# grant-froelich/Bathymetric-GNN

Measured on AMD Instinct MI355X. Metric: classified tile-nodes/s (fused graph build + 4-layer GAT forward + scatter), higher is better.
Workload: dtype f32

## Files before the change

bathymetric-gnn_amd/csrc/bgnn_api.hip:

```cpp
#include <stdarg.h>
#include <string.h>
#include <stdlib.h>

#include <algorithm>
#include <cmath>

#include "bgnn_internal.h"

namespace bgnn {

static thread_local char g_err[1024] = "";

void set_error(const char *fmt, ...) {
  va_list ap;
  va_start(ap, fmt);
  vsnprintf(g_err, sizeof(g_err), fmt, ap);
  va_end(ap);
}

int DevPool::alloc(size_t bytes, void **out) {
  if (bytes == 0) bytes = 256;
  bytes = (bytes + 255) & ~(size_t)255;
  auto it = free_blocks.lower_bound(bytes);
  if (it != free_blocks.end() && it->first <= bytes + bytes / 4 + 4096) {
// ... 211 lines not shown
    }
    c->owns_stream = true;
  }
  if (hipMalloc((void **)&c->zero_page, 16384) != hipSuccess || hipMemset(c->zero_page, 0, 16384) != hipSuccess) {
    set_error("zero page allocation failed");
    delete c;
    return BGNN_ERR_NOMEM;
  }
  c->stamps = reinterpret_cast<unsigned long long *>(c->zero_page + 1024);
  {
    auto env_int = [](const char *name, int dflt) { const char *e = getenv(name); return e ? atoi(e) : dflt; };
    BgnnOpts &o = c->opts;
    o.matrix_path = getenv("BGNN_BF16") ? 3 : getenv("BGNN_SPLIT_F16") ? 2 : getenv("BGNN_SPLIT_BF16") ? 1 : 0;
    o.fused = getenv("BGNN_NO_FUSED") ? 0 : 1;
    o.fold_extractor = getenv("BGNN_NO_FOLD") ? 0 : 1;
    o.ragged_atlas = getenv("BGNN_NO_ATLAS") ? 0 : 1;
    o.fused_front = getenv("BGNN_NO_FUSED_FRONT") ? 0 : 1;
    o.bf16_two_phase = getenv("BGNN_NO_TWO_PHASE") ? 0 : env_int("BGNN_TWO_PHASE", 1);
    o.bf16_layer0_af = getenv("BGNN_NO_LAYER0_AF") ? 0 : 1;
    o.stats_narrow = env_int("BGNN_STATS_NARROW", -1);
    o.diag_mask = env_int("BGNN_FUSED_DBG", 0);
    o.diag_stamps = getenv("BGNN_FUSED_STAMPS") ? 1 : 0;
    o.gemm_diag = env_int("BGNN_GEMM_DBG", 0);
    o.gemm_pair_major = getenv("BGNN_NO_PAIR_MAJOR") ? 0 : 1;
  }
  *out = c;
  return BGNN_OK;
}

static int *option_slot(bgnn_ctx *ctx, const char *name) {
  BgnnOpts &o = ctx->opts;
  struct { const char *n; int *p; } tab[] = {
      {"matrix_path", &o.matrix_path}, {"fused", &o.fused}, {"fold_extractor", &o.fold_extractor}, {"ragged_atlas", &o.ragged_atlas}, {"features_tiled", &o.features_tiled}, {"fused_front", &o.fused_front}, {"bf16_two_phase", &o.bf16_two_phase}, {"bf16_layer0_af", &o.bf16_layer0_af}, {"stats_narrow", &o.stats_narrow},
      {"diag_mask", &o.diag_mask}, {"diag_stamps", &o.diag_stamps}, {"gemm_diag", &o.gemm_diag}, {"gemm_pair_major", &o.gemm_pair_major}};
  for (auto &t : tab) if (strcmp(t.n, name) == 0) return t.p;
  return nullptr;
}

int bgnn_ctx_set_option(bgnn_ctx *ctx, const char *name, int value) {
  BGNN_REQUIRE(ctx && name, "bgnn_ctx_set_option: NULL argument");
  int *p = option_slot(ctx, name);
  BGNN_REQUIRE(p, "bgnn_ctx_set_option: unknown option '%s'", name);
  if (p == &ctx->opts.matrix_path) BGNN_REQUIRE(value >= 0 && value <= 3, "matrix_path=%d (0 exact f32, 1 bf16x3, 2 fp16x3, 3 bf16 storage)", value);
  if ((p == &ctx->opts.diag_mask || p == &ctx->opts.diag_stamps || p == &ctx->opts.gemm_diag) && value != 0)
    BGNN_REQUIRE(BGNN_DIAG, "option '%s' needs the diagnostic build of the library (python __graft_entry__.py --diag)", name);
  *p = value;
  return BGNN_OK;
}

int bgnn_ctx_get_option(bgnn_ctx *ctx, const char *name, int *value) {
  BGNN_REQUIRE(ctx && name && value, "bgnn_ctx_get_option: NULL argument");
  int *p = option_slot(ctx, name);
  BGNN_REQUIRE(p, "bgnn_ctx_get_option: unknown option '%s'", name);
  *value = *p;
  return BGNN_OK;
}

int bgnn_debug_stamps(bgnn_ctx *ctx, unsigned long long *out32) {
  if (!ctx || !out32) return BGNN_ERR_INVALID;
  (void)hipStreamSynchronize(ctx->stream);
  if (hipMemcpy(out32, ctx->stamps, 512, hipMemcpyDeviceToHost) != hipSuccess) return BGNN_ERR_HIP;
  (void)hipMemset(ctx->stamps, 0, 512);
  return BGNN_OK;
}

int bgnn_ctx_destroy(bgnn_ctx *ctx) {
  if (!ctx) return BGNN_OK;
// ... 285 lines not shown
```

bathymetric-gnn_amd/csrc/bgnn_internal.h:

```cpp
#pragma once
#include <hip/hip_runtime.h>
#include <stdint.h>
#include <stdio.h>
#include <string>
#include <cstdlib>
#include <vector>
#include <map>
#include <set>
#include <atomic>

#include "../../include/bgnn.h"
#include "../../include/bgnn_train.h"
#include "../../include/bgnn_optim.h"
#include "model_images.h"
#include "graph_plan.h"

namespace bgnn {

void set_error(const char *fmt, ...);

#define BGNN_HIP_CHECK(expr)                                                          \
  do {                                                                                \
    hipError_t _e = (expr);                                                           \
    if (_e != hipSuccess) {                                                           \
// ... 17 lines not shown
    if (_r != BGNN_OK) return _r; \
  } while (0)

struct DevPool {
  std::multimap<size_t, void *> free_blocks;
  std::map<void *, size_t> live;
  size_t total_bytes = 0;
  int alloc(size_t bytes, void **out);
  void release(void *p);
  void trim();
};

struct ProfRecord {
  int kernel;
  hipEvent_t start, stop;
};

}

struct BgnnOpts {
  int matrix_path = 0;
  int fused = 1;
  int fold_extractor = 1;
  int bf16_two_phase = 1;
  int bf16_layer0_af = 1;
  int stats_narrow = -1;
  int fused_front = 1;
  int features_tiled = 1;
  int ragged_atlas = 1;
  int diag_mask = 0;
  int diag_stamps = 0;
  int gemm_diag = 0;
  int gemm_pair_major = 1;
};

#ifndef BGNN_DIAG
#define BGNN_DIAG 0
#endif

struct bgnn_ctx {
  int device = 0;
  BgnnOpts opts;
  hipStream_t stream = nullptr;
  bool owns_stream = false;
  bgnn::DevPool pool;
  uint32_t prof_mask = 0;
  std::vector<bgnn::ProfRecord> prof_records;
  std::vector<hipEvent_t> event_pool;
  void *ws[7] = {nullptr, nullptr, nullptr, nullptr, nullptr, nullptr, nullptr};
  size_t ws_bytes[7] = {0, 0, 0, 0, 0, 0, 0};
  struct Staging { void *p; size_t cap; hipEvent_t ev; bool in_flight; };
  std::vector<Staging> staging;
  struct TableCache { int32_t n_tiles, h, w, item_cells; double rx, ry; BgnnTileMeta *d_tiles; BgnnWorkItem *d_items; int32_t n_items; uint64_t stamp; uint64_t id; int32_t refs; };
  std::vector<TableCache> table_cache;
  uint64_t table_stamp = 0, table_next_id = 1;
  std::set<struct bgnn_graph *> live_graphs;
  int num_cus = 256;
  float *zero_page = nullptr;
  unsigned long long *stamps = nullptr;
};

struct BgnnLayer {
  int d_in, heads, width;
  int concat;
  float *Wt;
  float *Wt_blk = nullptr;
// ... 272 lines not shown
```

bathymetric-gnn_amd/csrc/gat_layer_fused.hip:

```cpp
#include <stdlib.h>
#include <algorithm>
#include <type_traits>
#include <utility>
#include "gat_tile_common.h"

namespace bgnn {

typedef float f32x16 __attribute__((ext_vector_type(16)));

enum { EPI_NEXT = 0, EPI_HEADS = 1 };

#if BGNN_DIAG
#define DBG(bit) (a.dbg & (bit))
#define BGNN_STAMP(slot)                                                                   \
  if (a.stamps) {                                                                          \
    const unsigned long long _t = __builtin_amdgcn_s_memtime();                            \
    t_sum[slot] += _t - t_prev;                                                            \
    t_prev = _t;                                                                           \
  }
#else
#define DBG(bit) false
#define BGNN_STAMP(slot)
#endif

// ... 298 lines not shown
template <int KB0, int NB, bool ZERO, bool TAILZ>
__device__ __forceinline__ void agg_blocks(f32x16 &d, uint32_t tr0, uint32_t tr1, uint32_t bq, int hl) {
  u32x2 a0[NB], a1[NB];
  u32x4 b[NB];
#pragma unroll
  for (int i = 0; i < NB; ++i) {
    if (KB0 + i == 0) { a0[i] = lds_read_tr<0>(tr0); a1[i] = lds_read_tr<0>(tr1); b[i] = lds_read4u<0>(bq); }
    if (KB0 + i == 1) { a0[i] = lds_read_tr<1024>(tr0); a1[i] = lds_read_tr<1024>(tr1); b[i] = lds_read4u<32>(bq); }
    if (KB0 + i == 2) { a0[i] = lds_read_tr<2048>(tr0); a1[i] = lds_read_tr<2048>(tr1); b[i] = lds_read4u<64>(bq); }
    if (KB0 + i == 3) { a0[i] = lds_read_tr<3072>(tr0); a1[i] = lds_read_tr<3072>(tr1); b[i] = lds_read4u<96>(bq); }
    if (KB0 + i == 4) { a0[i] = lds_read_tr<4096>(tr0); a1[i] = lds_read_tr<4096>(tr1); b[i] = lds_read4u<128>(bq); }
    if (KB0 + i == 5) { a0[i] = lds_read_tr<5120>(tr0); a1[i] = lds_read_tr<5120>(tr1); b[i] = lds_read4u<160>(bq); }
    if (KB0 + i == 6) { a0[i] = lds_read_tr<6144>(tr0); a1[i] = lds_read_tr<6144>(tr1); b[i] = lds_read4u<192>(bq); }
    if (KB0 + i == 7) { a0[i] = lds_read_tr<7168>(tr0); a1[i] = lds_read_tr<7168>(tr1); b[i] = lds_read4u<224>(bq); }
  }
  lds_reads_done();
#pragma unroll
  for (int i = 0; i < NB; ++i) {
    if (TAILZ && KB0 + i == 7) {
      const u32x4 z4 = {0u, 0u, 0u, 0u};
      if (hl) b[i] = z4;
    }
    const u32x4 av = {a0[i].x, a0[i].y, a1[i].x, a1[i].y};
    const bf16x8 A = __builtin_bit_cast(bf16x8, av), B = __builtin_bit_cast(bf16x8, b[i]);
    if (ZERO && i == 0) {
      const f32x16 z = {0.f, 0.f, 0.f, 0.f, 0.f, 0.f, 0.f, 0.f, 0.f, 0.f, 0.f, 0.f, 0.f, 0.f, 0.f, 0.f};
      d = __builtin_amdgcn_mfma_f32_32x32x16_bf16(A, B, z, 0, 0, 0);
    } else {
      d = __builtin_amdgcn_mfma_f32_32x32x16_bf16(A, B, d, 0, 0, 0);
    }
  }
}

template <int HC, int C, int K, int NT, int EPI, int SP>
struct FusedLds {
  static constexpr int H = HC / C, NC = NT * 32, HR = FusedGeom<K>::HR;
  static constexpr int XB = SP == 3 ? 2 : 4;
  static constexpr int SLAB1 = HR * 32 * XB / 4;
  static constexpr int RING = SP == 3 && NT == 8 && EPI == EPI_NEXT ? 1 : 0;
  static constexpr bool DBUF = RING == 1, WDB = RING == 2;
  static constexpr int SLAB = DBUF ? 2 * SLAB1 : SLAB1;
  static constexpr int WBUF = (WDB ? 4 : 2) * WHalf<NT, SP>::BYTES / 4;
  static constexpr int PATCH_PAD = EPI == EPI_NEXT && SLAB + WBUF < 4 * 32 * TILED_PITCH ? 4 * 32 * TILED_PITCH - SLAB - WBUF : 0;
  static constexpr int HEADW = 96 + 6 * 32 + 8;
  static constexpr bool HAS_IN_ALPHA = SP == 3, HEADW_LATE = SP == 3 && EPI == EPI_HEADS, HID_IN_ALPHA = DBUF || WDB, ATT_LATE = DBUF || WDB;
  static constexpr int ATT_OFF = SLAB1 + 128 > 4 * 32 * TILED_PITCH ? SLAB1 + 128 : 4 * 32 * TILED_PITCH;
  static constexpr int RA = HAS_IN_ALPHA ? 0 : HR * (H + 1), RB = 2 * HC + (EPI == EPI_NEXT ? (ATT_LATE ? 0 : 2 * NC) : HEADW_LATE ? 0 : HEADW);
  static constexpr int RSZ = RA > RB ? RA : RB;
  static constexpr int APITCH = (H * (K + 1)) | 1;
  static constexpr int ALPHA = SP == 3 ? 4 * 32 * AggWindow<K>::PITCH / 4 : 128 * APITCH;
  static_assert(!HAS_IN_ALPHA || HR * (H + 1) + (HID_IN_ALPHA ? HR : 0) <= ALPHA, "the alpha_src and depth tables (and the halo ids) fit the dense-alpha region");
  static_assert(!DBUF || (4 * 32 * TILED_PITCH <= ATT_OFF && ATT_OFF + 2 * NC <= SLAB), "patches | att vectors share the slab region");
  static_assert(!WDB || (4 * 32 * TILED_PITCH <= ATT_OFF && ATT_OFF + 2 * NC <= SLAB + WBUF / 2), "patches | att vectors fit slab + W chunk buffer 0");
  static_assert(!HEADW_LATE || HEADW <= SLAB, "the heads' weight table fits the slab region");
  static_assert(SP != 3 || !AggWindow<K>::TAIL_BEYOND_PITCH || WBUF * 4 >= 8 * 64, "the 8 rows read past the slab image stay inside the W buffer");
  static constexpr int PRE = SLAB + WBUF + PATCH_PAD + RSZ + (HID_IN_ALPHA ? 128 : HR) + 4;
  static constexpr int ALIGN = (4 - PRE % 4) % 4;
  static constexpr int FLOATS = PRE + ALIGN + ALPHA;
  static constexpr bool WIDE_PHASE_A = K == 16 && EPI == EPI_HEADS && SP == 0;
  static constexpr int PER_CU = FLOATS * 4 * 3 <= 160 * 1024 && NT <= 3 && !WIDE_PHASE_A ? 3 : FLOATS * 4 * 2 <= 160 * 1024 ? 2 : 1;
};

template <int HC, int C, int K, int NT, int EPI, int SP = 0, int AGG = 0>
__global__ __launch_bounds__(256, (AGG != 0 && K == 16 ? 2 : FusedLds<HC, C, K, NT, EPI, SP>::PER_CU)) void gat_layer_fused_kernel(FusedArgs a) {
  static_assert(AGG == 0 || (SP == 0 && EPI == EPI_NEXT), "the plain backbones run on the exact path, layer form");
  static_assert(AGG != 2 || HC == 2 * C, "GraphSAGE: two virtual heads");
  constexpr int SRCW = AGG == 2 ? C : HC;
  constexpr int NTH = 256;
  constexpr int H = HC / C;
  constexpr int NC = NT * 32;
  constexpr int NSLAB = HC / 32, SPH = C / 32;
  constexpr bool GATHER_PIPE = SP == 0 && K <= 8 && EPI == EPI_NEXT && AGG == 0;
  using Geo = FusedGeom<K>;
  using Lds = FusedLds<HC, C, K, NT, EPI, SP>;
  constexpr int HR = Geo::HR, HW_ = Geo::HW, RAD = Geo::R;
  constexpr int XB = Lds::XB;
  constexpr int ROWB = 32 * XB;
  constexpr int CPR = ROWB / 16;
  using Off = StencilOffsets<K>;
  extern __shared__ __attribute__((aligned(128))) float lds[];
  float *slab = lds;
  float *wbuf = slab + Lds::SLAB;
  constexpr bool DBUF = Lds::DBUF, WDB = Lds::WDB;
  constexpr int SLAB1B = Lds::SLAB1 * 4;
  constexpr int RSZ = Lds::RSZ, APITCH = Lds::APITCH;
  float *rreg = wbuf + Lds::WBUF + Lds::PATCH_PAD;
  float *scsh = rreg;
  float *attr = Lds::HEADW_LATE ? slab : Lds::ATT_LATE ? slab + Lds::ATT_OFF : rreg + 2 * HC;
  int *cid = reinterpret_cast<int *>(rreg + RSZ);
  int *minid = cid + (Lds::HID_IN_ALPHA ? 128 : HR);
  float *alx = reinterpret_cast<float *>(minid + 4) + Lds::ALIGN;
  float *has = Lds::HAS_IN_ALPHA ? alx : rreg;
  float *hdp = has + HR * H;
  int *hid = Lds::HID_IN_ALPHA ? reinterpret_cast<int *>(alx + HR * (H + 1)) : reinterpret_cast<int *>(rreg + RSZ);

#if BGNN_DIAG
  unsigned long long t_sum[12] = {0, 0, 0, 0, 0, 0, 0, 0, 0, 0, 0, 0};
  unsigned long long t_prev = a.stamps ? __builtin_amdgcn_s_memtime() : 0;
  const unsigned long long t_clk0 = t_prev, t_real0 = a.stamps ? __builtin_amdgcn_s_memrealtime() : 0;
#endif
  const BlockPos pos = decode_block<FT_H>(a.tb);
  const int tid = threadIdx.x, lane = tid & 63;
  const int wave = __builtin_amdgcn_readfirstlane(tid >> 6);
  const int r = lane & 31, hl = lane >> 5;
  const int cell = wave * 32 + r;
  const int tr = cell / TILE_W, tc = cell % TILE_W;
  const int self_idx = (tr + RAD) * HW_ + tc + RAD;

  stage_w_half<NT, SP>(a.Wt, wbuf, 0, wave, lane);
  stage_w_half<NT, SP>(a.Wt, wbuf, 1, wave, lane);
// ... 32 lines not shown
  const uint32_t cell_m = cell_index(gr_m, gc_m);
  const int raw_m = node_at(cell_m);
  int tile_m = pos.tile;
  if (a.tile_of_cell) {
    const int t_ = *reinterpret_cast<const int *>(reinterpret_cast<const char *>(a.tile_of_cell) + (cell_m << 2));
    tile_m = raw_m >= 0 ? t_ : 0;
  }
  static_assert(NTH % CPR == 0, "pieces advance by whole halo rows");
  constexpr int RSTEP = NTH / CPR, RSTEP_R = RSTEP / HW_, RSTEP_C = RSTEP % HW_;
  int drow[NPIECE], prow_r[NPIECE], prow_c[NPIECE];
  {
    const int row0 = tid / CPR;
    int pr = row0 / HW_, pc = row0 - pr * HW_;
#pragma unroll
    for (int p = 0; p < NPIECE; ++p) {
      prow_r[p] = pr; prow_c[p] = pc;
      drow[p] = node_at(cell_index(pos.r0 + pr - RAD, pos.c0 + pc - RAD));
      pr += RSTEP_R; pc += RSTEP_C;
      if (pc >= HW_) { pc -= HW_; pr += 1; }
    }
  }
  constexpr int NSC = (HC + NTH - 1) / NTH;
  float scv[NSC], shv[NSC];
#pragma unroll
  for (int i = 0; i < NSC; ++i) {
    const int c = tid + i * NTH;
    scv[i] = c < HC ? a.scale[c] : 0.0f; shv[i] = c < HC ? a.shift[c] : 0.0f;
  }
  float vpre[NHL][3];
#pragma unroll
  for (int i = 0; i < NHL; ++i) {
    const int hh = hl + i * 2;
#pragma unroll
    for (int f = 0; f < 3; ++f) vpre[i][f] = (AGG == 0 && hh < H) ? a.V[hh * 3 + f] : 0.0f;
  }
  BGNN_STAMP(9)
  int hid_v = (tid < HR && in_tile(gr_h, gc_h) && raw_h >= 0) ? raw_h : -1;
  int my_pre = (!DBG(32) && in_tile(gr_m, gc_m)) ? raw_m : -1;
#pragma unroll
  for (int p = 0; p < NPIECE; ++p) {
    const bool row_ok = (p + 1) * NTH <= HR * CPR || prow_r[p] < FT_H + 2 * RAD;
    if (!(row_ok && in_tile(pos.r0 + prow_r[p] - RAD, pos.c0 + prow_c[p] - RAD))) drow[p] = -1;
  }
#if BGNN_DIAG
  if (a.stamps) asm volatile("" ::"v"(hid_v), "v"(my_pre), "v"(drow[0]));
#endif
  BGNN_STAMP(10)
  if (a.cell_map) {
    const bool wave_any = __builtin_amdgcn_ballot_w64(my_pre >= 0) != 0;
    if (lane == 0) minid[wave] = wave_any ? 1 : 0;
    __syncthreads();
    if ((minid[0] | minid[1] | minid[2] | minid[3]) == 0) {
      __builtin_amdgcn_s_waitcnt(0);
      return;
    }
  }
  float eraw[K], adv[NHL], hasv[H], hdep;
  float4 tdist;
  if constexpr (AGG != 0) {
    const uint64_t hrow = (uint32_t)(hid_v >= 0 ? hid_v : 0);
#pragma unroll
    for (int hh = 0; hh < H; ++hh) hasv[hh] = 0.0f;
    if constexpr (AGG == 1) hasv[0] = a.asd[hrow];
#pragma unroll
    for (int i = 0; i < K; ++i) eraw[i] = 0.0f;
#pragma unroll
    for (int i = 0; i < NHL; ++i) adv[i] = 0.0f;
    hdep = 0.0f; tdist = make_float4(0.f, 0.f, 0.f, 0.f);
  } else {
    const uint64_t hrow = (uint32_t)(hid_v >= 0 ? hid_v : 0), mrow = (uint32_t)(my_pre >= 0 ? my_pre : 0);
    hdep = a.node_depth[hrow];
    tdist = a.tile_dist[tile_m];
    if constexpr (H % 4 == 0) {
#pragma unroll
      for (int q = 0; q < H / 4; ++q) {
        const float4 v4 = *reinterpret_cast<const float4 *>(a.asd + hrow * 2 * H + 4 * q);
        hasv[4 * q] = v4.x; hasv[4 * q + 1] = v4.y; hasv[4 * q + 2] = v4.z; hasv[4 * q + 3] = v4.w;
      }
    } else {
#pragma unroll
      for (int hh = 0; hh < H; ++hh) hasv[hh] = a.asd[hrow * 2 * H + hh];
    }
    const float4 *ep = reinterpret_cast<const float4 *>(a.slope + mrow * K);
#pragma unroll
    for (int i = 0; i < K / 4; ++i) {
      const float4 q = ep[i];
      eraw[4 * i] = q.x; eraw[4 * i + 1] = q.y; eraw[4 * i + 2] = q.z; eraw[4 * i + 3] = q.w;
    }
#pragma unroll
    for (int i = 0; i < NHL; ++i) {
      const int hh = hl + i * 2;
      adv[i] = hh < H ? a.asd[mrow * 2 * H + H + hh] : 0.0f;
    }
  }
  static_assert(HW_ % 2 == 0, "row parity follows the halo column");
  auto swz = [](int row) { return XB == 4 ? ((row % HW_) >> 1) & 7 : (row >> 2) & 3; };
  static_assert(NSLAB * ROWB <= 4096, "the zero page covers a whole block's worth of slab offsets");
  const char *xbase = reinterpret_cast<const char *>(a.xw);
  const char *zp = reinterpret_cast<const char *>(a.zero_page);
  const char *dbase[NPIECE];
  {
    const int cc = tid % CPR;
#pragma unroll
    for (int p = 0; p < NPIECE; ++p) {
      const int row = prow_r[p] * HW_ + prow_c[p];
      const int c = cc ^ swz(row);
      dbase[p] = drow[p] >= 0 ? xbase + ((uint64_t)(uint32_t)drow[p] * (uint32_t)(SRCW * XB) + (uint32_t)(c * 16)) : zp;
    }
  }
  int npc = 0;
#pragma unroll
  for (int p = 0; p < NPIECE; ++p) npc += (p * NTH + wave * 64 < HR * CPR) ? 1 : 0;
  static_assert(Lds::HEADW % 4 == 0 && Lds::HEADW <= 128 * 4, "the heads' table is at most two wave pieces");
  auto stage_head_table = [&]() {
    if constexpr (EPI == EPI_HEADS) {
      if (wave < 2 && (wave * 64 + lane) * 4 < Lds::HEADW)
        __builtin_amdgcn_global_load_lds(reinterpret_cast<const void *>(a.hd_tab + (wave * 64 + lane) * 4),
                                         (__attribute__((address_space(3))) void *)(attr + wave * 256), 16, 0, 0);
    }
  };
  auto issue_slab = [&](int s) {
    const int sb = (AGG == 2 ? s % SPH : s) * ROWB;
#pragma unroll
    for (int p = 0; p < NPIECE; ++p) {
      if ((p + 1) * NTH <= HR * CPR || p * NTH + tid < HR * CPR) {
        __builtin_amdgcn_global_load_lds(reinterpret_cast<const void *>(dbase[p] + sb),
                                         (__attribute__((address_space(3))) void *)(slab + (DBUF && !(s & 1) ? Lds::SLAB1 : 0) + (p * NTH + wave * 64) * 4), 16, 0, 0);
      }
    }
  };
  if (tid < HR) {
    hid[tid] = hid_v;
#pragma unroll
    for (int hh = 0; hh < H; ++hh) has[hh * HR + tid] = hid_v >= 0 ? hasv[hh] : (AGG == 0 ? -__builtin_inff() : 0.0f);
    hdp[tid] = hid_v >= 0 ? hdep : 0.0f;
  }
  if (Lds::HID_IN_ALPHA && hl == 0) cid[cell] = my_pre < 0 ? -1 : my_pre;
  {
    float sink = 0.0f;
#pragma unroll
    for (int i = 0; i < NHL; ++i) sink += adv[i];
#pragma unroll
    for (int i = 0; i < K; ++i) sink += eraw[i];
#pragma unroll
    for (int hh = 0; hh < H; ++hh) sink += hasv[hh];
    sink += hdep + tdist.x + tdist.y + tdist.z;
    asm volatile("" ::"v"(sink));
  }
  BGNN_STAMP(11)
  issue_slab(0);
  BGNN_STAMP(0)
  wait_lgkm0();
  __builtin_amdgcn_s_barrier();
  BGNN_STAMP(1)

  uint32_t apk[NHL][(K + 2) / 2];
#pragma unroll
  for (int i = 0; i < NHL; ++i)
#pragma unroll
    for (int b = 0; b < (K + 2) / 2; ++b) apk[i][b] = 0u;
  {
    const uint32_t hid0 = lds_addr(hid), has0 = lds_addr(has);
    int self_a = self_idx;
    if constexpr (K == 16 && EPI == EPI_HEADS && SP == 3) {
      int t2 = threadIdx.x;
      asm volatile("" : "+v"(t2));
      const int c2 = (t2 & 31) | (t2 >> 6) << 5;
      self_a = (c2 / TILE_W + RAD) * HW_ + c2 % TILE_W + RAD;
    }
    int my = lds_read1i<0>(hid0 + (uint32_t)self_a * 4u);
    lds_reads_done();
    if (DBG(32)) my = -1;
    float part[NHL][K + 1];
    if (my < 0) {
#pragma unroll
      for (int i = 0; i < NHL; ++i)
#pragma unroll
        for (int b = 0; b <= K; ++b) part[i][b] = 0.0f;
    } else {
      using S = HaloSlot<K, HW_>;
      int nb[K];
      float hs[NHL][K + 1];
      halo_ids<K, HW_>(hid0 + (uint32_t)(self_a - S::MAXOFF) * 4u, nb, std::make_integer_sequence<int, K>{});
      if constexpr (AGG != 0) {
        static_assert(AGG == 0 || NHL == 1, "one (virtual) head per lane");
        if constexpr (AGG == 1) halo_alpha_src<1, K, HW_>(has0 + (uint32_t)(self_a - S::MAXOFF) * 4u, hs[0], std::make_integer_sequence<int, K>{});
        lds_reads_done();
        int cnt = a.self_loops ? 1 : 0;
#pragma unroll
        for (int b = 0; b < K; ++b) cnt += nb[b] >= 0 ? 1 : 0;
        const float inv = 1.0f / (float)(cnt > 0 ? cnt : 1);
#pragma unroll
        for (int b = 0; b <= K; ++b) {
// ... 1 lines not shown
          float c;
          if constexpr (AGG == 1) c = self ? hs[0][K] * hs[0][K] : (on ? hs[0][b] * hs[0][K] : 0.0f);
          else if constexpr (AGG == 2) c = hl == 0 ? ((self ? a.self_loops != 0 : on) ? inv : 0.0f) : (self ? 1.0f : 0.0f);
          else c = self ? (a.self_loops ? 2.0f : 1.0f) : (on ? 1.0f : 0.0f);
          part[0][b] = c;
        }
      } else {
#pragma unroll
      for (int i = 0; i < NHL; ++i) {
        const int hh = hl + i * 2 < H ? hl + i * 2 : 0;
        halo_alpha_src<H, K, HW_>(has0 + (uint32_t)(hh * HR + self_a - S::MAXOFF) * 4u, hs[i], std::make_integer_sequence<int, K>{});
      }
      float dsrc[K + 1];
      halo_depths<K, HW_>(lds_addr(hdp) + (uint32_t)(self_a - S::MAXOFF) * 4u, dsrc, std::make_integer_sequence<int, K>{});
      lds_reads_done();
      EdgeTerms<K> et;
      edge_terms_compact<K>(nb, eraw, dsrc, tdist.x, tdist.y, tdist.z, et);
      if constexpr (NHL == 2 && H % 2 == 0 && H >= 4) {
        attention_head_pair<K, false>(et, hs[0], hs[1], adv[0], adv[1], vpre[0], vpre[1], part[0], part[1]);
      } else {
#pragma unroll
        for (int i = 0; i < NHL; ++i)
          if (hl + i * 2 < H) attention_head<K, false>(et, hs[i], adv[i], vpre[i], part[i]);
      }
      }
    }
#pragma unroll
    for (int i = 0; i < NHL; ++i) {
      const int hh = hl + i * 2;
      if (hh < H) {
        if constexpr (SP == 3) {
#pragma unroll
          for (int b = 0; b <= K; b += 2) apk[i][b / 2] = pack_bf16x2(part[i][b], b + 1 <= K ? part[i][b + 1] : 0.0f);
        } else {
          lds_write_coefficients<K>(lds_addr(alx + cell * APITCH + hh * (K + 1)), part[i], std::make_integer_sequence<int, K + 1>{});
        }
      }
    }
  }

  BGNN_STAMP(2)
  f32x16 acc[NT];
  if constexpr (SP != 0 || BGNN_DIAG) {
#pragma unroll
    for (int t = 0; t < NT; ++t)
#pragma unroll
      for (int i = 0; i < 16; ++i) acc[t][i] = 0.0f;
  }

  const uint32_t slab0 = lds_addr(slab);
  const uint32_t wbuf0 = lds_addr(wbuf + 4 * hl * NC + r * WTileGroup<NT>::TG);
  constexpr bool F32_CHUNKS = SP == 0 || SP == 3;
  constexpr uint32_t CX1 = F32_CHUNKS ? 32 : 16, CX2 = 64, CX3 = F32_CHUNKS ? 96 : 80;
  const uint32_t scsh0 = lds_addr(scsh) + (F32_CHUNKS ? hl * 16 : hl * 32);
  const uint32_t wsp0 = lds_addr(wbuf) + lane * 16;
  const uint32_t alx0 = lds_addr(alx + cell * APITCH);
  constexpr uint32_t WHALF = WHalf<NT, SP>::BYTES;
  using Win = AggWindow<K>;
  const int wbase = Win::base(wave);
  const uint32_t dn0 = lds_addr(alx) + wave * (32 * Win::PITCH);
  const uint32_t bq0 = dn0 + r * Win::PITCH + hl * 16;
  uint32_t tr0 = 0, tr1 = 0;
  if constexpr (SP == 3) {
    const int grp = lane >> 4, q = (lane >> 2) & 3, p4 = lane & 3, cb = grp & 1;
    const int row0 = wbase + 8 * hl + q;
    const int c = 2 * cb + (p4 >> 1);
    tr0 = slab0 + row0 * 64 + ((c ^ ((row0 >> 2) & 3)) << 4) + 8 * (p4 & 1);
    tr1 = slab0 + (row0 + 4) * 64 + ((c ^ (((row0 + 4) >> 2) & 3)) << 4) + 8 * (p4 & 1);
  }

  {
#pragma unroll 1
    for (int s = 0; s < NSLAB; ++s) {
      const uint32_t slabs = slab0;
      constexpr int WH = WHalf<NT, SP>::PER_WAVE;
      constexpr int WREM = WHalf<NT, SP>::NQ % 4;
      const bool wextra = wave < WREM;
      auto densify = [&](int hd) {
        if (hd == 0) {
          const u32x4 z4 = {0u, 0u, 0u, 0u};
          constexpr int DB = 32 * Win::PITCH;
#pragma unroll
          for (int i = 0; i < (DB + 1023) / 1024; ++i)
            if ((i + 1) * 1024 <= DB || lane * 16 + i * 1024 < DB)
              asm volatile("ds_write_b128 %0, %1" ::"v"(dn0 + lane * 16 + i * 1024), "v"(z4) : "memory");
        }
        if (hl == (hd & 1)) {
          const int wself = self_idx - wbase;
          const uint32_t rowb = dn0 + r * Win::PITCH;
#pragma unroll
          for (int b = 0; b <= K; ++b) {
            const int off = b < K ? Off::dr[b < K ? b : 0] * HW_ + Off::dc[b < K ? b : 0] : 0;
            const int wp = wself - off;
            const uint32_t ad = rowb + (uint32_t)wp * 2u;
            const uint32_t v = NHL > 1 && (hd >> 1) ? apk[NHL > 1 ? 1 : 0][b / 2] : apk[0][b / 2];
            if (b & 1) asm volatile("ds_write_b16_d16_hi %0, %1" ::"v"(ad), "v"(v) : "memory");
            else asm volatile("ds_write_b16 %0, %1" ::"v"(ad), "v"(v) : "memory");
          }
        }
      };
      if constexpr (SP == 3) {
        if (s % SPH == 0 && s > 0) densify(s / SPH);
      }
      if (s == 0 || WDB) wait_vm_lgkm<0>();
// ... 861 lines not shown
  };
  col_pass(std::integral_constant<int, 0>{}); col_pass(std::integral_constant<int, 1>{});
  col_pass(std::integral_constant<int, 2>{}); col_pass(std::integral_constant<int, 3>{});
  {
    float srow[H2], drow_[H2];
#pragma unroll
    for (int hd = 0; hd < H2; ++hd) {
      const float sl = sl_[hd], dl = dl_[hd];
      srow[hd] = sl + __shfl_xor(sl, 32);
      drow_[hd] = dl + __shfl_xor(dl, 32);
    }
    if (id >= 0 && hl == 0) {
      float *ao = a.asd_out + (int64_t)id * 2 * H2;
      *reinterpret_cast<float4 *>(ao) = make_float4(srow[0], srow[1], srow[2], srow[3]);
      *reinterpret_cast<float4 *>(ao + 4) = make_float4(drow_[0], drow_[1], drow_[2], drow_[3]);
    }
  }
}

template <int K, bool AF = false>
static int launch_two_phase(bgnn_ctx *ctx, const FusedArgs &a) {
  constexpr size_t lds_bytes = (size_t)TwoPhaseLds<K>::BYTES;
  static std::atomic<uint64_t> configured{0};
  auto kern = gat_layer_bf16_2p_kernel<K, AF>;
  if (!(configured.load(std::memory_order_relaxed) >> (ctx->device & 63) & 1)) {
    BGNN_HIP_CHECK(hipFuncSetAttribute(reinterpret_cast<const void *>(kern), hipFuncAttributeMaxDynamicSharedMemorySize, (int)lds_bytes));
    configured.fetch_or(1ull << (ctx->device & 63), std::memory_order_relaxed);
  }
  hipLaunchKernelGGL(kern, dim3(a.tb.n_blocks), dim3(256), lds_bytes, ctx->stream, a);
  BGNN_HIP_CHECK(hipGetLastError());
  return BGNN_OK;
}

template <int HC, int C, int K, int NT, int EPI, int SP = 0, int AGG = 0>
static int launch_inst(bgnn_ctx *ctx, const FusedArgs &a) {
  constexpr size_t lds_bytes = (size_t)FusedLds<HC, C, K, NT, EPI, SP>::FLOATS * 4;
  static_assert(lds_bytes <= 160 * 1024, "one workgroup fits the CU's LDS");
  static std::atomic<uint64_t> configured{0};
  auto kern = gat_layer_fused_kernel<HC, C, K, NT, EPI, SP, AGG>;
  if (!(configured.load(std::memory_order_relaxed) >> (ctx->device & 63) & 1)) {
    BGNN_HIP_CHECK(hipFuncSetAttribute(reinterpret_cast<const void *>(kern), hipFuncAttributeMaxDynamicSharedMemorySize, (int)lds_bytes));
    configured.fetch_or(1ull << (ctx->device & 63), std::memory_order_relaxed);
  }
  hipLaunchKernelGGL(kern, dim3(a.tb.n_blocks), dim3(256), lds_bytes, ctx->stream, a);
  BGNN_HIP_CHECK(hipGetLastError());
  return BGNN_OK;
}

template <int HC, int NT, int EPI>
static int launch_by_stencil(bgnn_ctx *ctx, const bgnn_graph *g, int sp, const FusedArgs &a) {
  switch (sp) {
    case 0:
      return g->K == 8 ? launch_inst<HC, 64, 8, NT, EPI, 0>(ctx, a) : g->K == 4 ? launch_inst<HC, 64, 4, NT, EPI, 0>(ctx, a)
                                                                                 : launch_inst<HC, 64, 16, NT, EPI, 0>(ctx, a);
    case 3:
      return g->K == 8 ? launch_inst<HC, 64, 8, NT, EPI, 3>(ctx, a) : g->K == 4 ? launch_inst<HC, 64, 4, NT, EPI, 3>(ctx, a)
                                                                                 : launch_inst<HC, 64, 16, NT, EPI, 3>(ctx, a);
    default: break;
  }
  if (g->K == 16) return BGNN_ERR_UNSUPPORTED;
  if (sp == 1) return g->K == 8 ? launch_inst<HC, 64, 8, NT, EPI, 1>(ctx, a) : launch_inst<HC, 64, 4, NT, EPI, 1>(ctx, a);
  return g->K == 8 ? launch_inst<HC, 64, 8, NT, EPI, 2>(ctx, a) : launch_inst<HC, 64, 4, NT, EPI, 2>(ctx, a);
}

static bool fused_supported(const bgnn_graph *g, int C) {
  return g->kind == 0 && (g->K == 4 || g->K == 8 || g->K == 16) && g->n_blocks3 > 0 && C == 64 && g->max_w <= 8192 && g->compact_edges;
}

static void fill_common(FusedArgs &a, const bgnn_graph *g, const BgnnLayer &L, const float *V3, const void *xw, const float *asd, int relu) {
  a.tb.tiles = g->d_tiles; a.tb.items2 = g->uni_h ? nullptr : g->d_items3;
  a.tb.bh = g->bh3; a.tb.bw = g->bw3; a.tb.n_blocks = g->n_blocks3;
  a.node_id = g->d_node_id; a.cell_map = nullptr; a.tile_of_cell = nullptr;
  if (g->d_atlas) {
    a.tb.tiles = g->d_atlas_tile; a.tb.items2 = nullptr;
    a.tb.bh = g->atlas_h / 8; a.tb.bw = g->atlas_w / 16; a.tb.n_blocks = a.tb.bh * a.tb.bw;
    a.node_id = g->d_atlas; a.cell_map = g->d_cell_of_node; a.tile_of_cell = g->d_atlas_tile_of;
  }
  a.xw = xw; a.asd = asd; a.V = V3 ? V3 : L.V; a.scale = L.scale; a.shift = L.shift;
  a.slope = g->d_slope; a.node_depth = g->d_node_depth; a.tile_dist = g->d_tile_dist;
  a.relu = relu; a.zero_page = g->ctx->zero_page; a.dump = g->ctx->zero_page + 2048;
  a.dbg = BGNN_DIAG ? g->ctx->opts.diag_mask : 0;
  a.stamps = BGNN_DIAG && g->ctx->opts.diag_stamps ? g->ctx->stamps : nullptr;
}

int launch_fused_layer_next(bgnn_ctx *ctx, const bgnn_graph *g, const BgnnLayer &L, const BgnnLayer &Ln, int C, const float *V3,
                            const void *xw, const float *asd, void *xw_next, float *asd_next) {
  if (!fused_supported(g, C) || (!g->edge_default && !V3)) return BGNN_ERR_UNSUPPORTED;
  const int HC = L.heads * C, NC = Ln.heads * C;
  if (Ln.d_in != HC) return BGNN_ERR_UNSUPPORTED;
  FusedArgs a{};
  fill_common(a, g, L, V3, xw, asd, L.concat ? 1 : 0);
  int split = ctx->opts.matrix_path;
  if (split == 2 && !Ln.Wsp16) split = 1;
  a.Wt = split == 3 ? Ln.Wbf : split == 2 ? Ln.Wsp16 : split == 1 ? Ln.Wsp : Ln.Wfp;
  a.w_inv = Ln.Wsp16_inv;
  a.att_src = Ln.att_src; a.att_dst = Ln.att_dst; a.out = xw_next; a.asd_out = asd_next;
  a.H2 = Ln.heads; a.C2 = C;
  ProfScope ps(ctx, BGNN_K_FUSED);
  const bool main_shape = (HC == 256 && NC == 256) || (HC == 256 && NC == 64);
  if (split == 3 && !main_shape) return BGNN_ERR_UNSUPPORTED;
  if ((split == 1 || split == 2) && (!main_shape || g->K == 16)) { split = 0; a.Wt = Ln.Wfp; }
  if (split == 3 && HC == 256 && NC == 256 && C == 64 && ctx->opts.bf16_two_phase)
    return g->K == 8 ? launch_two_phase<8>(ctx, a) : g->K == 4 ? launch_two_phase<4>(ctx, a) : launch_two_phase<16>(ctx, a);
#define BGNN_FUSED_CASE(hc, nt) if (HC == hc && NC == nt * 32) return launch_by_stencil<hc, nt, EPI_NEXT>(ctx, g, split, a);
  BGNN_FUSED_CASE(256, 8) BGNN_FUSED_CASE(256, 2)
#undef BGNN_FUSED_CASE
  if (g->K == 16) return BGNN_ERR_UNSUPPORTED;
#define BGNN_FUSED_CASE(hc, nt)                                                                         \
  if (HC == hc && NC == nt * 32)                                                                        \
    return g->K == 8 ? launch_inst<hc, 64, 8, nt, EPI_NEXT>(ctx, a) : launch_inst<hc, 64, 4, nt, EPI_NEXT>(ctx, a);
  BGNN_FUSED_CASE(128, 4) BGNN_FUSED_CASE(128, 2) BGNN_FUSED_CASE(64, 2)
#undef BGNN_FUSED_CASE
  return BGNN_ERR_UNSUPPORTED;
}

int launch_fused_layer0_af(bgnn_ctx *ctx, const bgnn_graph *g, const BgnnLayer &L, const BgnnLayer &Ln, int C, const float *V3,
                           const void *h1, const float *asd, const float *W0af, const float *shift_af, void *xw_next, float *asd_next) {
  if (!fused_supported(g, C) || (!g->edge_default && !V3) || !W0af || !shift_af) return BGNN_ERR_UNSUPPORTED;
  if (C != 64 || L.heads != 4 || Ln.heads != 4 || Ln.d_in != 256 || !Ln.Wbf) return BGNN_ERR_UNSUPPORTED;
  FusedArgs a{};
  fill_common(a, g, L, V3, h1, asd, L.concat ? 1 : 0);
  a.shift = shift_af;
  a.Wt = Ln.Wbf; a.W0af = W0af;
  a.att_src = Ln.att_src; a.att_dst = Ln.att_dst; a.out = xw_next; a.asd_out = asd_next;
  a.H2 = Ln.heads; a.C2 = C;
  ProfScope ps(ctx, BGNN_K_FUSED);
  return g->K == 8 ? launch_two_phase<8, true>(ctx, a) : g->K == 4 ? launch_two_phase<4, true>(ctx, a) : launch_two_phase<16, true>(ctx, a);
}

int launch_fused_plain_layer(bgnn_ctx *ctx, const bgnn_graph *g, int mode, int C, const float *x, const float *dinv, const float *Wfp,
                             const float *ones, const float *post_scale, const float *post_shift, int post_relu, float *out) {
  if (!fused_supported(g, C) || !Wfp || mode < 1 || mode > 3) return BGNN_ERR_UNSUPPORTED;
  FusedArgs a{};
  BgnnLayer L{};
  L.V = nullptr; L.scale = const_cast<float *>(ones); L.shift = ctx->zero_page;
  fill_common(a, g, L, nullptr, x, dinv, 0);
  a.Wt = Wfp; a.att_src = post_scale; a.att_dst = post_shift; a.out = out; a.asd_out = nullptr;
  a.H2 = 1; a.C2 = C; a.relu2 = post_relu; a.self_loops = g->include_self_loops;
  ProfScope ps(ctx, BGNN_K_FUSED);
#define BGNN_PLAIN_CASE(M, HCV)                                                                                   \
  if (mode == M)                                                                                                  \
    return g->K == 8 ? launch_inst<HCV, 64, 8, 2, EPI_NEXT, 0, M>(ctx, a) : g->K == 4 ? launch_inst<HCV, 64, 4, 2, EPI_NEXT, 0, M>(ctx, a) \
                                                                                       : launch_inst<HCV, 64, 16, 2, EPI_NEXT, 0, M>(ctx, a);
// ... 36 lines not shown
```

bathymetric-gnn_amd/runtime.py:

```python
from __future__ import annotations

import ctypes as C
import os
import threading
from typing import Dict, Optional

import numpy as np
import torch

_PKG_DIR = os.path.dirname(os.path.abspath(__file__))
LIB_PATH = os.path.join(_PKG_DIR, "libbgnn_hip.so")

K_NAMES = ["scan", "stats", "features", "export", "gemm", "attcoef", "aggregate", "heads", "scatter", "fused"]
K_INDEX = {n: i for i, n in enumerate(K_NAMES)}

NODE_FEATURE_IDS = {"depth": 0, "local_mean": 1, "local_std": 2, "gradient_x": 3, "gradient_y": 4,
                    "gradient_magnitude": 5, "curvature": 6, "uncertainty": 7}
EDGE_FEATURE_IDS = {"distance": 0, "depth_difference": 1, "slope": 2}
EF_ZERO = 3

ERR_INVALID, ERR_HIP, ERR_NOMEM, ERR_UNSUPPORTED = -1, -2, -3, -4
ABI_VERSION = 7
MATRIX_PATHS = {"exact_f32": 0, "bf16x3": 1, "fp16x3": 2, "bf16": 3}
OPTION_NAMES = ("matrix_path", "fused", "fold_extractor", "ragged_atlas", "features_tiled", "fused_front",
                "bf16_two_phase", "bf16_layer0_af", "stats_narrow", "diag_mask", "diag_stamps",
                "gemm_diag", "gemm_pair_major")


GNN_TYPES = {"GAT": 0, "GCN": 1, "GraphSAGE": 2, "GIN": 3}


class ModelDesc(C.Structure):
    _fields_ = [("in_channels", C.c_int32), ("hidden", C.c_int32), ("num_layers", C.c_int32),
                ("heads", C.c_int32), ("num_classes", C.c_int32), ("edge_dim", C.c_int32),
                ("predict_correction", C.c_int32), ("bn_eps", C.c_float), ("gnn_type", C.c_int32)]


class Tiles(C.Structure):
    _fields_ = [("n_tiles", C.c_int32), ("hw", C.POINTER(C.c_int32)), ("resolution", C.POINTER(C.c_double)),
                ("depth", C.c_void_p), ("mask", C.c_void_p), ("uncertainty", C.c_void_p)]


class GraphOpts(C.Structure):
    _fields_ = [("connectivity", C.c_int32), ("include_self_loops", C.c_int32),
                ("n_node_features", C.c_int32), ("node_features", C.c_int32 * 8),
                ("n_edge_features", C.c_int32), ("edge_features", C.c_int32 * 4)]


class Outputs(C.Structure):
    _fields_ = [("class_logits", C.c_void_p), ("class_probs", C.c_void_p), ("predicted_class", C.c_void_p),
                ("confidence", C.c_void_p), ("correction", C.c_void_p), ("action", C.c_void_p),
                ("needs_review", C.c_void_p), ("auto_correct", C.c_void_p), ("hidden", C.c_void_p)]


class Dropout(C.Structure):
    _fields_ = [("p_extractor", C.c_float), ("p_attention", C.c_float), ("p_features", C.c_float), ("p_heads", C.c_float),
                ("seed", C.c_uint64)]


# ... 453 lines not shown
```

Before: 308.9 million.

## Add light-form exact fused GAT kernel with half-width slab and four blocks per CU

Adds a 'light form' variant of the exact-f32 fused GAT layer kernel for narrow next stages (NT<=3, K<=8). It stages half-width slab rows (64 bytes) and processes each slab in two half steps with a new swizzle. It stores at most two heads' attention coefficients in LDS, keeping the extra head's coefficients in registers until needed. The smaller LDS footprint is meant to allow four workgroups per CU and raise occupancy. The cost is more barriers and half-step passes per slab, plus extra register pressure. It is on by default via a new option, and an LDS-size query entry point is added.

```diff
diff --git a/bathymetric-gnn_amd/csrc/bgnn_api.hip b/bathymetric-gnn_amd/csrc/bgnn_api.hip
--- a/bathymetric-gnn_amd/csrc/bgnn_api.hip
+++ b/bathymetric-gnn_amd/csrc/bgnn_api.hip
@@ -267,7 +267,7 @@
   BgnnOpts &o = ctx->opts;
   struct { const char *n; int *p; } tab[] = {
       {"matrix_path", &o.matrix_path}, {"fused", &o.fused}, {"fold_extractor", &o.fold_extractor}, {"ragged_atlas", &o.ragged_atlas}, {"features_tiled", &o.features_tiled}, {"fused_front", &o.fused_front}, {"bf16_two_phase", &o.bf16_two_phase}, {"bf16_layer0_af", &o.bf16_layer0_af}, {"stats_narrow", &o.stats_narrow},
-      {"diag_mask", &o.diag_mask}, {"diag_stamps", &o.diag_stamps}, {"gemm_diag", &o.gemm_diag}, {"gemm_pair_major", &o.gemm_pair_major}};
+      {"diag_mask", &o.diag_mask}, {"diag_stamps", &o.diag_stamps}, {"gemm_diag", &o.gemm_diag}, {"gemm_pair_major", &o.gemm_pair_major}, {"fused_light_form", &o.fused_light_form}};
   for (auto &t : tab) if (strcmp(t.n, name) == 0) return t.p;
   return nullptr;
 }
diff --git a/bathymetric-gnn_amd/csrc/bgnn_internal.h b/bathymetric-gnn_amd/csrc/bgnn_internal.h
--- a/bathymetric-gnn_amd/csrc/bgnn_internal.h
+++ b/bathymetric-gnn_amd/csrc/bgnn_internal.h
@@ -73,6 +73,7 @@
   int diag_stamps = 0;
   int gemm_diag = 0;
   int gemm_pair_major = 1;
+  int fused_light_form = 1;
 };
 
 #ifndef BGNN_DIAG
diff --git a/bathymetric-gnn_amd/csrc/gat_layer_fused.hip b/bathymetric-gnn_amd/csrc/gat_layer_fused.hip
--- a/bathymetric-gnn_amd/csrc/gat_layer_fused.hip
+++ b/bathymetric-gnn_amd/csrc/gat_layer_fused.hip
@@ -354,11 +354,15 @@
   }
 }
 
-template <int HC, int C, int K, int NT, int EPI, int SP>
+template <int HC, int C, int K, int NT, int EPI, int SP, int LF = 0>
 struct FusedLds {
   static constexpr int H = HC / C, NC = NT * 32, HR = FusedGeom<K>::HR;
   static constexpr int XB = SP == 3 ? 2 : 4;
-  static constexpr int SLAB1 = HR * 32 * XB / 4;
+  static constexpr bool HS = LF != 0;
+  static_assert(!HS || (SP == 0 && K <= 8 && NT <= 3), "light form: exact f32, halo of one cell, narrow next stage");
+  static constexpr int AW = HS && H > 2 ? 2 : H;
+  static_assert(H <= 2 * AW, "light form: two head pairs at the most");
+  static constexpr int SLAB1 = HS ? HR * 16 : HR * 32 * XB / 4;
   static constexpr int RING = SP == 3 && NT == 8 && EPI == EPI_NEXT ? 1 : 0;
   static constexpr bool DBUF = RING == 1, WDB = RING == 2;
   static constexpr int SLAB = DBUF ? 2 * SLAB1 : SLAB1;
@@ -369,7 +373,7 @@
   static constexpr int ATT_OFF = SLAB1 + 128 > 4 * 32 * TILED_PITCH ? SLAB1 + 128 : 4 * 32 * TILED_PITCH;
   static constexpr int RA = HAS_IN_ALPHA ? 0 : HR * (H + 1), RB = 2 * HC + (EPI == EPI_NEXT ? (ATT_LATE ? 0 : 2 * NC) : HEADW_LATE ? 0 : HEADW);
   static constexpr int RSZ = RA > RB ? RA : RB;
-  static constexpr int APITCH = (H * (K + 1)) | 1;
+  static constexpr int APITCH = (AW * (K + 1)) | 1;
   static constexpr int ALPHA = SP == 3 ? 4 * 32 * AggWindow<K>::PITCH / 4 : 128 * APITCH;
   static_assert(!HAS_IN_ALPHA || HR * (H + 1) + (HID_IN_ALPHA ? HR : 0) <= ALPHA, "the alpha_src and depth tables (and the halo ids) fit the dense-alpha region");
   static_assert(!DBUF || (4 * 32 * TILED_PITCH <= ATT_OFF && ATT_OFF + 2 * NC <= SLAB), "patches | att vectors share the slab region");
@@ -380,11 +384,12 @@
   static constexpr int ALIGN = (4 - PRE % 4) % 4;
   static constexpr int FLOATS = PRE + ALIGN + ALPHA;
   static constexpr bool WIDE_PHASE_A = K == 16 && EPI == EPI_HEADS && SP == 0;
-  static constexpr int PER_CU = FLOATS * 4 * 3 <= 160 * 1024 && NT <= 3 && !WIDE_PHASE_A ? 3 : FLOATS * 4 * 2 <= 160 * 1024 ? 2 : 1;
+  static constexpr int PER_CU = HS && FLOATS * 4 * 4 <= 160 * 1024 ? 4 : FLOATS * 4 * 3 <= 160 * 1024 && NT <= 3 && !WIDE_PHASE_A ? 3 : FLOATS * 4 * 2 <= 160 * 1024 ? 2 : 1;
 };
 
-template <int HC, int C, int K, int NT, int EPI, int SP = 0, int AGG = 0>
-__global__ __launch_bounds__(256, (AGG != 0 && K == 16 ? 2 : FusedLds<HC, C, K, NT, EPI, SP>::PER_CU)) void gat_layer_fused_kernel(FusedArgs a) {
+template <int HC, int C, int K, int NT, int EPI, int SP = 0, int AGG = 0, int LF = 0>
+__global__ __launch_bounds__(256, (AGG != 0 && K == 16 ? 2 : FusedLds<HC, C, K, NT, EPI, SP, LF>::PER_CU)) void gat_layer_fused_kernel(FusedArgs a) {
+  static_assert(LF == 0 || AGG == 0, "light form: GAT instances");
   static_assert(AGG == 0 || (SP == 0 && EPI == EPI_NEXT), "the plain backbones run on the exact path, layer form");
   static_assert(AGG != 2 || HC == 2 * C, "GraphSAGE: two virtual heads");
   constexpr int SRCW = AGG == 2 ? C : HC;
@@ -394,10 +399,11 @@
   constexpr int NSLAB = HC / 32, SPH = C / 32;
   constexpr bool GATHER_PIPE = SP == 0 && K <= 8 && EPI == EPI_NEXT && AGG == 0;
   using Geo = FusedGeom<K>;
-  using Lds = FusedLds<HC, C, K, NT, EPI, SP>;
+  using Lds = FusedLds<HC, C, K, NT, EPI, SP, LF>;
+  constexpr bool HS = Lds::HS;
   constexpr int HR = Geo::HR, HW_ = Geo::HW, RAD = Geo::R;
   constexpr int XB = Lds::XB;
-  constexpr int ROWB = 32 * XB;
+  constexpr int ROWB = HS ? 64 : 32 * XB;
   constexpr int CPR = ROWB / 16;
   using Off = StencilOffsets<K>;
   extern __shared__ __attribute__((aligned(128))) float lds[];
@@ -496,7 +502,10 @@
   for (int i = 0; i < NHL; ++i) {
     const int hh = hl + i * 2;
 #pragma unroll
-    for (int f = 0; f < 3; ++f) vpre[i][f] = (AGG == 0 && hh < H) ? a.V[hh * 3 + f] : 0.0f;
+    for (int f = 0; f < 3; ++f) {
+      if constexpr (HS && H == 1) vpre[i][f] = a.V[f];
+      else vpre[i][f] = (AGG == 0 && hh < H) ? a.V[hh * 3 + f] : 0.0f;
+    }
   }
   BGNN_STAMP(9)
   int hid_v = (tid < HR && in_tile(gr_h, gc_h) && raw_h >= 0) ? raw_h : -1;
@@ -558,18 +567,23 @@
     }
   }
   static_assert(HW_ % 2 == 0, "row parity follows the halo column");
-  auto swz = [](int row) { return XB == 4 ? ((row % HW_) >> 1) & 7 : (row >> 2) & 3; };
+  auto swz = [](int row) {
+    return HS ? (((row % HW_) >> 2) & 1) | (((row / HW_) & 1) << 1) : XB == 4 ? ((row % HW_) >> 1) & 7 : (row >> 2) & 3;
+  };
   static_assert(NSLAB * ROWB <= 4096, "the zero page covers a whole block's worth of slab offsets");
   const char *xbase = reinterpret_cast<const char *>(a.xw);
   const char *zp = reinterpret_cast<const char *>(a.zero_page);
   const char *dbase[NPIECE];
+  constexpr bool DB32 = HS && H == 1;
+  uint32_t doff[NPIECE];
   {
     const int cc = tid % CPR;
 #pragma unroll
     for (int p = 0; p < NPIECE; ++p) {
       const int row = prow_r[p] * HW_ + prow_c[p];
-      const int c = cc ^ swz(row);
+      const int c = cc ^ (HS ? ((prow_c[p] >> 2) & 1) | ((prow_r[p] & 1) << 1) : swz(row));
       dbase[p] = drow[p] >= 0 ? xbase + ((uint64_t)(uint32_t)drow[p] * (uint32_t)(SRCW * XB) + (uint32_t)(c * 16)) : zp;
+      doff[p] = drow[p] >= 0 ? (uint32_t)drow[p] * (uint32_t)(SRCW * XB / 16) + (uint32_t)c : ~0u;
     }
   }
   int npc = 0;
@@ -588,7 +602,10 @@
 #pragma unroll
     for (int p = 0; p < NPIECE; ++p) {
       if ((p + 1) * NTH <= HR * CPR || p * NTH + tid < HR * CPR) {
-        __builtin_amdgcn_global_load_lds(reinterpret_cast<const void *>(dbase[p] + sb),
+        uint32_t dof = doff[p];
+        if constexpr (DB32) asm volatile("" : "+v"(dof));
+        const char *src = DB32 ? (dof != ~0u ? xbase + ((uint64_t)dof << 4) : zp) : dbase[p];
+        __builtin_amdgcn_global_load_lds(reinterpret_cast<const void *>(src + sb),
                                          (__attribute__((address_space(3))) void *)(slab + (DBUF && !(s & 1) ? Lds::SLAB1 : 0) + (p * NTH + wave * 64) * 4), 16, 0, 0);
       }
     }
@@ -623,6 +640,10 @@
   for (int i = 0; i < NHL; ++i)
 #pragma unroll
     for (int b = 0; b < (K + 2) / 2; ++b) apk[i][b] = 0u;
+  static_assert(!HS || NHL <= 2, "light form: a lane holds at most one head beside the one in the table");
+  float keep[K + 1];
+#pragma unroll
+  for (int b = 0; b <= K; ++b) keep[b] = 0.0f;
   {
     const uint32_t hid0 = lds_addr(hid), has0 = lds_addr(has);
     int self_a = self_idx;
@@ -690,8 +711,11 @@
         if constexpr (SP == 3) {
 #pragma unroll
           for (int b = 0; b <= K; b += 2) apk[i][b / 2] = pack_bf16x2(part[i][b], b + 1 <= K ? part[i][b + 1] : 0.0f);
+        } else if (HS && H > Lds::AW && i > 0) {
+#pragma unroll
+          for (int b = 0; b <= K; ++b) keep[b] = part[i][b];
         } else {
-          lds_write_coefficients<K>(lds_addr(alx + cell * APITCH + hh * (K + 1)), part[i], std::make_integer_sequence<int, K + 1>{});
+          lds_write_coefficients<K>(lds_addr(alx + cell * APITCH + (HS && H > Lds::AW ? hl : hh) * (K + 1)), part[i], std::make_integer_sequence<int, K + 1>{});
         }
       }
     }
@@ -727,7 +751,97 @@
     tr1 = slab0 + (row0 + 4) * 64 + ((c ^ (((row0 + 4) >> 2) & 3)) << 4) + 8 * (p4 & 1);
   }
 
-  {
+  if constexpr (HS) {
+    constexpr int AW = Lds::AW;
+    auto half_step = [&](auto hc_, int s, uint32_t ap, f32x4 (&g)[4]) {
+      constexpr int h = decltype(hc_)::value;
+      const int hs = 2 * s + h;
+      wait_vm_lgkm<0>();
+      __builtin_amdgcn_s_barrier();
+      if (h == 0 && s == 0) {
+#pragma unroll
+        for (int i = 0; i < NSC; ++i) {
+          const int c = tid + i * NTH;
+          if (c < HC) { scsh[c] = scv[i]; scsh[HC + c] = shv[i]; }
+        }
+        if constexpr (EPI == EPI_HEADS) stage_head_table();
+        if (EPI == EPI_NEXT && wave < 2 && lane * 4 < NC)
+          __builtin_amdgcn_global_load_lds(reinterpret_cast<const void *>((wave == 0 ? a.att_src : a.att_dst) + lane * 4),
+                                           (__attribute__((address_space(3))) void *)(attr + wave * NC), 16, 0, 0);
+        wait_lgkm0();
+        __builtin_amdgcn_s_barrier();
+      }
+      if (hs >= 1 && hs + 1 < 2 * NSLAB) stage_w_half<NT, SP>(a.Wt, wbuf, hs + 1, wave, lane);
+      constexpr int jA = 2 * h, jB = 2 * h + 1;
+      g[jA] = (f32x4){0.f, 0.f, 0.f, 0.f}; g[jB] = (f32x4){0.f, 0.f, 0.f, 0.f};
+      auto row_addr = [&](int b) -> uint32_t {
+        const int dr_ = b < K ? Off::dr[b < K ? b : 0] : 0, dc_ = b < K ? Off::dc[b < K ? b : 0] : 0;
+        const int nidx = self_idx - dr_ * HW_ - dc_;
+        const int hcol = tc + RAD - dc_, hline = tr + RAD - dr_;
+        return slab0 + nidx * 64 + ((((((hcol >> 2) & 1) | ((hline & 1) << 1))) ^ hl) << 4);
+      };
+      if constexpr (GATHER_PIPE) {
+        f32x4 xb[2][2];
+        float al[2];
+        auto issue = [&](int b, int q) {
+          const uint32_t rb = row_addr(b);
+          al[q] = lds_read1<0>(ap + 4 * b);
+          xb[q][0] = lds_read4<0>(rb); xb[q][1] = lds_read4<0>(rb ^ 32);
+        };
+        issue(0, 0);
+#pragma unroll
+        for (int b = 0; b <= K; ++b) {
+          const int q = b & 1;
+          if (b + 1 <= K) { issue(b + 1, q ^ 1); lds_reads_wait<3>(); } else lds_reads_done();
+          g[jA] += al[q] * xb[q][0]; g[jB] += al[q] * xb[q][1];
+        }
+      } else {
+#pragma unroll
+        for (int b = 0; b <= K; ++b) {
+          const uint32_t rb = row_addr(b);
+          const float alpha = lds_read1<0>(ap + 4 * b);
+          const f32x4 x0 = lds_read4<0>(rb), x1 = lds_read4<0>(rb ^ 32);
+          lds_reads_done();
+          g[jA] += alpha * x0; g[jB] += alpha * x1;
+        }
+      }
+      {
+        const uint32_t cp = scsh0 + s * 128 + h * 64;
+        const f32x4 sc0 = lds_read4<0>(cp), sc1 = lds_read4<32>(cp), sh0 = lds_read4<HC * 4>(cp), sh1 = lds_read4<HC * 4 + 32>(cp);
+        lds_reads_done();
+        g[jA] = g[jA] * sc0 + sh0;
+        g[jB] = g[jB] * sc1 + sh1;
+        if (a.relu) {
+#pragma unroll
+          for (int j = jA; j <= jB; ++j) {
+            asm("v_max_f32 %0, 0, %0" : "+v"(g[j].x)); asm("v_max_f32 %0, 0, %0" : "+v"(g[j].y));
+            asm("v_max_f32 %0, 0, %0" : "+v"(g[j].z)); asm("v_max_f32 %0, 0, %0" : "+v"(g[j].w));
+          }
+        }
+      }
+      wait_lgkm0();
+      __builtin_amdgcn_s_barrier();
+      if (hs + 1 < 2 * NSLAB) issue_slab(hs + 1);
+      if constexpr (h == 0) {
+        if (s == 0) MfmaGroups<NT, NC, 0, 4, true>::run(acc, g, wbuf0);
+        else MfmaGroups<NT, NC, 0, 4>::run(acc, g, wbuf0);
+      } else {
+        MfmaGroups<NT, NC, 4, 8>::run(acc, g, wbuf0);
+      }
+    };
+#pragma unroll 1
+    for (int s = 0; s < NSLAB; ++s) {
+      const int hd = s / SPH;
+      if constexpr (H > AW) {
+        if (s == AW * SPH && hl + AW < H)
+          lds_write_coefficients<K>(alx0 + hl * ((K + 1) * 4), keep, std::make_integer_sequence<int, K + 1>{});
+      }
+      const uint32_t ap = alx0 + (H > AW ? (hd & (AW - 1)) : hd) * ((K + 1) * 4);
+      f32x4 g[4];
+      half_step(std::integral_constant<int, 0>{}, s, ap, g);
+      half_step(std::integral_constant<int, 1>{}, s, ap, g);
+    }
+  } else {
 #pragma unroll 1
     for (int s = 0; s < NSLAB; ++s) {
       const uint32_t slabs = slab0;
@@ -1655,12 +1769,12 @@
   return BGNN_OK;
 }
 
-template <int HC, int C, int K, int NT, int EPI, int SP = 0, int AGG = 0>
+template <int HC, int C, int K, int NT, int EPI, int SP = 0, int AGG = 0, int LF = 0>
 static int launch_inst(bgnn_ctx *ctx, const FusedArgs &a) {
-  constexpr size_t lds_bytes = (size_t)FusedLds<HC, C, K, NT, EPI, SP>::FLOATS * 4;
+  constexpr size_t lds_bytes = (size_t)FusedLds<HC, C, K, NT, EPI, SP, LF>::FLOATS * 4;
   static_assert(lds_bytes <= 160 * 1024, "one workgroup fits the CU's LDS");
   static std::atomic<uint64_t> configured{0};
-  auto kern = gat_layer_fused_kernel<HC, C, K, NT, EPI, SP, AGG>;
+  auto kern = gat_layer_fused_kernel<HC, C, K, NT, EPI, SP, AGG, LF>;
   if (!(configured.load(std::memory_order_relaxed) >> (ctx->device & 63) & 1)) {
     BGNN_HIP_CHECK(hipFuncSetAttribute(reinterpret_cast<const void *>(kern), hipFuncAttributeMaxDynamicSharedMemorySize, (int)lds_bytes));
     configured.fetch_or(1ull << (ctx->device & 63), std::memory_order_relaxed);
@@ -1668,14 +1782,22 @@
   hipLaunchKernelGGL(kern, dim3(a.tb.n_blocks), dim3(256), lds_bytes, ctx->stream, a);
   BGNN_HIP_CHECK(hipGetLastError());
   return BGNN_OK;
+}
+
+template <int HC, int K, int NT, int EPI>
+static int launch_exact(bgnn_ctx *ctx, const FusedArgs &a) {
+  if constexpr (K <= 8 && NT <= 3) {
+    if (ctx->opts.fused_light_form) return launch_inst<HC, 64, K, NT, EPI, 0, 0, 1>(ctx, a);
+  }
+  return launch_inst<HC, 64, K, NT, EPI, 0>(ctx, a);
 }
 
 template <int HC, int NT, int EPI>
 static int launch_by_stencil(bgnn_ctx *ctx, const bgnn_graph *g, int sp, const FusedArgs &a) {
   switch (sp) {
     case 0:
-      return g->K == 8 ? launch_inst<HC, 64, 8, NT, EPI, 0>(ctx, a) : g->K == 4 ? launch_inst<HC, 64, 4, NT, EPI, 0>(ctx, a)
-                                                                                 : launch_inst<HC, 64, 16, NT, EPI, 0>(ctx, a);
+      return g->K == 8 ? launch_exact<HC, 8, NT, EPI>(ctx, a) : g->K == 4 ? launch_exact<HC, 4, NT, EPI>(ctx, a)
+                                                                           : launch_exact<HC, 16, NT, EPI>(ctx, a);
     case 3:
       return g->K == 8 ? launch_inst<HC, 64, 8, NT, EPI, 3>(ctx, a) : g->K == 4 ? launch_inst<HC, 64, 4, NT, EPI, 3>(ctx, a)
                                                                                  : launch_inst<HC, 64, 16, NT, EPI, 3>(ctx, a);
@@ -1684,6 +1806,23 @@
   if (g->K == 16) return BGNN_ERR_UNSUPPORTED;
   if (sp == 1) return g->K == 8 ? launch_inst<HC, 64, 8, NT, EPI, 1>(ctx, a) : launch_inst<HC, 64, 4, NT, EPI, 1>(ctx, a);
   return g->K == 8 ? launch_inst<HC, 64, 8, NT, EPI, 2>(ctx, a) : launch_inst<HC, 64, 4, NT, EPI, 2>(ctx, a);
+}
+
+template <int HC, int K, int NT, int EPI>
+static int exact_lds_bytes(int lf) {
+  if constexpr (K <= 8 && NT <= 3) {
+    if (lf) return FusedLds<HC, 64, K, NT, EPI, 0, 1>::FLOATS * 4;
+  }
+  return lf ? -1 : FusedLds<HC, 64, K, NT, EPI, 0, 0>::FLOATS * 4;
+}
+extern "C" int bgnn_internal_fused_lds_bytes(int hc, int k, int nt, int epi, int lf) {
+#define BGNN_LDS_CASE(HCV, KV, NTV, EPIV) if (hc == HCV && k == KV && nt == NTV && epi == EPIV) return exact_lds_bytes<HCV, KV, NTV, EPIV>(lf);
+#define BGNN_LDS_STENCILS(HCV, NTV, EPIV) BGNN_LDS_CASE(HCV, 4, NTV, EPIV) BGNN_LDS_CASE(HCV, 8, NTV, EPIV) BGNN_LDS_CASE(HCV, 16, NTV, EPIV)
+  BGNN_LDS_STENCILS(256, 8, EPI_NEXT) BGNN_LDS_STENCILS(256, 2, EPI_NEXT) BGNN_LDS_STENCILS(128, 4, EPI_NEXT)
+  BGNN_LDS_STENCILS(128, 2, EPI_NEXT) BGNN_LDS_STENCILS(64, 2, EPI_NEXT) BGNN_LDS_STENCILS(64, 3, EPI_HEADS)
+#undef BGNN_LDS_STENCILS
+#undef BGNN_LDS_CASE
+  return -1;
 }
 
 static bool fused_supported(const bgnn_graph *g, int C) {
@@ -1731,7 +1870,7 @@
   if (g->K == 16) return BGNN_ERR_UNSUPPORTED;
 #define BGNN_FUSED_CASE(hc, nt)                                                                         \
   if (HC == hc && NC == nt * 32)                                                                        \
-    return g->K == 8 ? launch_inst<hc, 64, 8, nt, EPI_NEXT>(ctx, a) : launch_inst<hc, 64, 4, nt, EPI_NEXT>(ctx, a);
+    return g->K == 8 ? launch_exact<hc, 8, nt, EPI_NEXT>(ctx, a) : launch_exact<hc, 4, nt, EPI_NEXT>(ctx, a);
   BGNN_FUSED_CASE(128, 4) BGNN_FUSED_CASE(128, 2) BGNN_FUSED_CASE(64, 2)
 #undef BGNN_FUSED_CASE
   return BGNN_ERR_UNSUPPORTED;
diff --git a/bathymetric-gnn_amd/runtime.py b/bathymetric-gnn_amd/runtime.py
--- a/bathymetric-gnn_amd/runtime.py
+++ b/bathymetric-gnn_amd/runtime.py
@@ -24,7 +24,7 @@
 MATRIX_PATHS = {"exact_f32": 0, "bf16x3": 1, "fp16x3": 2, "bf16": 3}
 OPTION_NAMES = ("matrix_path", "fused", "fold_extractor", "ragged_atlas", "features_tiled", "fused_front",
                 "bf16_two_phase", "bf16_layer0_af", "stats_narrow", "diag_mask", "diag_stamps",
-                "gemm_diag", "gemm_pair_major")
+                "gemm_diag", "gemm_pair_major", "fused_light_form")
 
 
 GNN_TYPES = {"GAT": 0, "GCN": 1, "GraphSAGE": 2, "GIN": 3}
```

Measured after the change: 312.1 million, median of 6. +1.0%, better.
